# rsasaki0109/lidarslam_ros2

Hardware: AMD Instinct MI355X
Metric: scan registrations/sec (30k-pt scan vs 10-frame submap) (higher is better)
Workload: dtype f32; 1 GPU; cfg2: single NDT align(), 30000-pt VLP-32 scan (vg 0.2) vs 10-frame submap (vg 0.1), ndt_resolution 5.0, DIRECT7, max_iterations 30, transformation_epsilon 0; 1018 different scans (stream of 64); target_points=661519, voxels_valid=643, derivative_passes_last_scan=242, parallelism=1 registration stream per GPU x1, collective=none (one rank)

## Files before the change

include/lidarslam_reg.h:

```cpp
#ifndef LIDARSLAM_REG_H
#define LIDARSLAM_REG_H

#include <stddef.h>
#include <stdint.h>

#ifdef __cplusplus
extern "C" {
#endif

typedef struct lsr_handle_s* lsr_handle;

typedef enum lsr_status {
  LSR_OK = 0,
  LSR_ERR_INVALID_ARGUMENT = -1,
  LSR_ERR_NO_DEVICE = -2,
  LSR_ERR_HIP = -3,
  LSR_ERR_NO_TARGET = -4,
  LSR_ERR_NO_SOURCE = -5,
  LSR_ERR_NOT_IMPLEMENTED = -6,
  LSR_ERR_INDEX_OVERFLOW = -7,
  LSR_ERR_TOO_FEW_POINTS = -8
} lsr_status;

typedef enum lsr_method { LSR_METHOD_NDT = 0, LSR_METHOD_GICP = 1 } lsr_method;
// ... 129 lines not shown
  double distance;
  const void* cloud;
  size_t n_points;
} lsr_submap;
typedef struct lsr_loop_params {
  double threshold_loop_closure_score;
  double distance_loop_closure;
  double range_of_searching_loop_closure;
  int search_submap_num;
  float voxel_leaf_size;
  int top_k;
  int reserved;
} lsr_loop_params;
typedef struct lsr_loop_edge {
  int id_from;
  int id_to;
  int accepted;
  int converged;
  int iterations;
  int n_target_points;
  double candidate_distance;
  double fitness_score;
  double relative_pose[16];
  float final_transformation[16];
} lsr_loop_edge;
int lsr_search_loop(lsr_handle h, const lsr_submap* submaps, int num_submaps, size_t stride_bytes, int on_device,
                    const lsr_loop_params* params, lsr_loop_edge* edges, int edge_capacity, int* n_evaluated);

int lsr_ndt_grid_info(lsr_handle h, int32_t* info8);
int lsr_ndt_grid_dump(lsr_handle h, int32_t* idx, int32_t* npts, double* mean, double* icov);
int lsr_ndt_grid_centroids(lsr_handle h, float* centroid);
int lsr_ndt_derivatives(lsr_handle h, const double* p6, const float* T16, int compute_hessian, double* score,
                        double* grad, double* hess);
int lsr_gicp_covariances(lsr_handle h, int which, double* cov);
int lsr_nearest_neighbors(lsr_handle h, const float* T16, int32_t* idx, float* d2);
int lsr_get_profile(lsr_handle h, lsr_profile* out, int reset);
int lsr_debug_angle_tables(const double* p6, int d1_sign, float* jang_ref, float* hang_ref, float* jang_tab, float* hang_tab);

#ifdef __cplusplus
}
#endif
#endif
```

lidarslam_ros2_amd/_capi.py:

```python
from __future__ import annotations

import ctypes as C
import os

_HERE = os.path.dirname(os.path.abspath(__file__))
LIB_PATH = os.path.join(_HERE, os.environ.get("LSR_LIB_NAME", "liblidarslam_reg.so"))

OK = 0
METHOD_NDT, METHOD_GICP = 0, 1
KDTREE, DIRECT26, DIRECT7, DIRECT1 = 0, 1, 2, 3
(RESOLUTION, TRANSFORMATION_EPSILON, STEP_SIZE, OUTLIER_RATIO, MAX_CORRESPONDENCE_DISTANCE, ROTATION_EPSILON,
 EUCLIDEAN_FITNESS_EPSILON, GICP_EPSILON) = range(8)
(MAX_ITERATIONS, NEIGHBORHOOD, NUM_THREADS, K_CORRESPONDENCES, MAX_INNER_ITERATIONS, RANSAC_ITERATIONS,
 HESSIAN_D1_SIGN, PROFILE, NDT_WORKGROUP, NDT_TABLE_MODE, GRID_BUILDER, WAIT_MODE, NDT_QUAD, _UNASSIGNED_45, VOXEL_FILTER_FORM, NDT_SPLIT, TARGET_PREPARED) = range(32, 49)

EXPORTED_SYMBOLS = [
    "lsr_version", "lsr_status_string", "lsr_last_error", "lsr_device_count", "lsr_create", "lsr_destroy",
    "lsr_set_f64", "lsr_set_i32", "lsr_get_f64", "lsr_get_i32", "lsr_set_input_target", "lsr_set_input_target_device",
    "lsr_set_input_target_frames", "lsr_set_input_source", "lsr_set_input_source_device", "lsr_set_input_source_filtered", "lsr_set_input_source_frontend", "lsr_voxel_grid_filter",
    "lsr_share_target", "lsr_wait_stream", "lsr_align", "lsr_align_batch",
    "lsr_get_final_transformation", "lsr_has_converged", "lsr_get_fitness_score", "lsr_search_loop", "lsr_ndt_grid_info",
    "lsr_ndt_grid_dump", "lsr_ndt_grid_centroids", "lsr_ndt_derivatives", "lsr_gicp_covariances", "lsr_nearest_neighbors", "lsr_get_profile",
    "lsr_debug_angle_tables", "lsr_set_input_source_pc2", "lsr_get_source_pc2", "lsr_voxel_grid_filter_pc2", "lsr_shard_range", "lsr_comm_unique_id", "lsr_comm_create", "lsr_comm_destroy", "lsr_align_batch_sharded",
    "lsr_shard_plan", "lsr_align_batch_planned", "lsr_align_fitness_batch",
    "lsr_set_input_target_batch", "lsr_set_input_source_batch", "lsr_get_fitness_score_batch", "lsr_set_input_target_bcast", "lsr_get_source_pc2_device",
    "lsr_comm_all_gather_records", "lsr_set_input_target_frames_filtered", "lsr_prepare_target",
]


class Result(C.Structure):
    _fields_ = [("converged", C.c_int32), ("iterations", C.c_int32), ("score", C.c_double),
                ("n_evaluations", C.c_int32), ("n_correspondences", C.c_int32), ("gpu_ms", C.c_double)]


class Profile(C.Structure):
    _fields_ = [("deriv_ms_total", C.c_double), ("deriv_launches", C.c_int64), ("deriv_points", C.c_int64),
                ("deriv_pairs", C.c_int64)]


class SubMap(C.Structure):
    _fields_ = [("position", C.c_double * 3), ("orientation", C.c_double * 4), ("distance", C.c_double),
                ("cloud", C.c_void_p), ("n_points", C.c_size_t)]


class LoopParams(C.Structure):
    _fields_ = [("threshold_loop_closure_score", C.c_double), ("distance_loop_closure", C.c_double),
                ("range_of_searching_loop_closure", C.c_double), ("search_submap_num", C.c_int),
                ("voxel_leaf_size", C.c_float), ("top_k", C.c_int), ("reserved", C.c_int)]


class LoopEdge(C.Structure):
    _fields_ = [("id_from", C.c_int), ("id_to", C.c_int), ("accepted", C.c_int), ("converged", C.c_int),
                ("iterations", C.c_int), ("n_target_points", C.c_int), ("candidate_distance", C.c_double),
                ("fitness_score", C.c_double), ("relative_pose", C.c_double * 16), ("final_transformation", C.c_float * 16)]

# ... 39 lines not shown
    L.lsr_destroy.argtypes = [vp]
    L.lsr_set_f64.argtypes = [vp, C.c_int, C.c_double]
    L.lsr_set_i32.argtypes = [vp, C.c_int, C.c_int]
    L.lsr_get_f64.argtypes = [vp, C.c_int, dp]
    L.lsr_get_i32.argtypes = [vp, C.c_int, ip]
    for name in ("lsr_set_input_target", "lsr_set_input_target_device", "lsr_set_input_source",
                 "lsr_set_input_source_device"):
        getattr(L, name).argtypes = [vp, vp, C.c_size_t, C.c_size_t]
    L.lsr_share_target.argtypes = [vp, vp]
    L.lsr_wait_stream.argtypes = [vp, vp]
    L.lsr_set_input_target_frames.argtypes = [vp, C.c_int, C.POINTER(vp), C.POINTER(C.c_size_t), C.c_size_t, fp, C.c_int]
    L.lsr_set_input_target_frames_filtered.argtypes = [vp, C.c_int, C.POINTER(vp), C.POINTER(C.c_size_t), C.c_size_t, fp, C.c_int, C.c_float,
                                                       C.POINTER(C.c_size_t)]
    L.lsr_prepare_target.argtypes = [vp]
    L.lsr_set_input_source_filtered.argtypes = [vp, vp, C.c_size_t, C.c_size_t, C.c_float, C.c_int, C.POINTER(C.c_size_t)]
    L.lsr_set_input_source_frontend.argtypes = [vp, vp, C.c_size_t, C.c_size_t, C.c_double, C.c_double, C.c_float, C.c_int,
                                                C.POINTER(C.c_size_t)]
    L.lsr_voxel_grid_filter.argtypes = [vp, vp, C.c_size_t, C.c_size_t, C.c_float, vp, C.c_size_t, C.c_size_t,
                                        C.POINTER(C.c_size_t)]
    L.lsr_align.argtypes = [vp, fp, fp, C.POINTER(Result), vp, C.c_size_t]
    L.lsr_align_batch.argtypes = [C.POINTER(vp), C.c_int, fp, fp, C.POINTER(Result)]
    L.lsr_get_final_transformation.argtypes = [vp, fp]
    L.lsr_has_converged.argtypes = [vp, ip]
    L.lsr_get_fitness_score.argtypes = [vp, C.c_double, dp]
    L.lsr_get_fitness_score_batch.argtypes = [C.POINTER(vp), C.c_int, C.c_double, dp]
    L.lsr_set_input_target_batch.argtypes = [C.POINTER(vp), C.c_int, C.POINTER(vp), C.POINTER(C.c_size_t), C.c_size_t, C.c_int]
    L.lsr_set_input_source_batch.argtypes = [C.POINTER(vp), C.c_int, C.POINTER(vp), C.POINTER(C.c_size_t), C.c_size_t, C.c_int]
    L.lsr_search_loop.argtypes = [vp, C.POINTER(SubMap), C.c_int, C.c_size_t, C.c_int, C.POINTER(LoopParams),
                                  C.POINTER(LoopEdge), C.c_int, ip]
    L.lsr_ndt_grid_info.argtypes = [vp, ip]
    L.lsr_ndt_grid_dump.argtypes = [vp, ip, ip, dp, dp]
    L.lsr_ndt_grid_centroids.argtypes = [vp, fp]
    L.lsr_ndt_derivatives.argtypes = [vp, dp, fp, C.c_int, dp, dp, dp]
    L.lsr_gicp_covariances.argtypes = [vp, C.c_int, dp]
    L.lsr_nearest_neighbors.argtypes = [vp, fp, ip, fp]
    L.lsr_get_profile.argtypes = [vp, C.POINTER(Profile), C.c_int]
    L.lsr_debug_angle_tables.argtypes = [dp, C.c_int, fp, fp, fp, fp]
    L.lsr_set_input_source_pc2.argtypes = [vp, vp, C.c_size_t, C.POINTER(Pc2Layout), C.c_double, C.c_double, C.c_float, C.c_int,
                                           C.POINTER(C.c_size_t)]
    L.lsr_get_source_pc2.argtypes = [vp, vp, C.c_size_t, C.POINTER(Pc2Layout), C.POINTER(C.c_size_t)]
    L.lsr_get_source_pc2_device.argtypes = [vp, vp, C.c_size_t, C.POINTER(Pc2Layout), C.POINTER(C.c_size_t)]
    L.lsr_voxel_grid_filter_pc2.argtypes = [vp, vp, C.c_size_t, C.POINTER(Pc2Layout), C.c_float, vp, C.c_size_t, C.POINTER(Pc2Layout),
                                            C.POINTER(C.c_size_t)]
    L.lsr_shard_range.argtypes = [C.c_int, C.c_int, C.c_int, ip, ip]
    L.lsr_shard_range.restype = None
    L.lsr_comm_unique_id.argtypes = [vp]
    L.lsr_comm_create.argtypes = [vp, C.c_int, C.c_int, C.c_int, C.POINTER(vp)]
    L.lsr_comm_destroy.argtypes = [vp]
    L.lsr_align_batch_sharded.argtypes = [vp, C.POINTER(vp), C.c_int, C.c_int, fp, C.c_int, C.POINTER(ShardRecord)]
    L.lsr_set_input_target_bcast.argtypes = [vp, vp, vp, C.c_size_t, C.c_size_t, C.c_int, C.c_int]
    L.lsr_align_fitness_batch.argtypes = [C.POINTER(vp), C.c_int, fp, fp, C.POINTER(Result), C.c_double, dp]
    i32p = C.POINTER(C.c_int32)
    L.lsr_shard_plan.argtypes = [C.c_int, dp, C.c_int, i32p, i32p, i32p]
    L.lsr_align_batch_planned.argtypes = [vp, C.POINTER(vp), C.c_int, C.c_int, i32p, i32p, fp, C.c_int, C.POINTER(ShardRecord)]
    for name in EXPORTED_SYMBOLS:
        fn = getattr(L, name)
        if fn.restype is C.c_int or name not in ("lsr_version", "lsr_status_string", "lsr_last_error"):
            if name not in ("lsr_version", "lsr_status_string", "lsr_last_error", "lsr_shard_range"):
                fn.restype = C.c_int
    _lib = L
    return L


def check(status: int, where: str) -> None:
    if status != OK:
        raise RegistrationError(status, where)
# ... 1 lines not shown
```

lidarslam_ros2_amd/csrc/capi.hip:

```cpp
#include <algorithm>
#include <chrono>
#include <functional>
#include <limits>
#include <cmath>
#include <cstdlib>
#include <mutex>
#include <numeric>
#include <thread>

#include "handle.hpp"

namespace lsr {
static thread_local std::string g_last_error;
void set_last_error(const std::string& s) { g_last_error = s; }
}

using namespace lsr;

namespace {

#define LSR_CHECK_HANDLE(h)                      \
  if (!(h)) {                                    \
    set_last_error("null handle");               \
    return LSR_ERR_INVALID_ARGUMENT;             \
// ... 562 lines not shown
    return LSR_OK;
  };
  const std::function<int()> poll_hook = [&]() { return eager_dispatch(false); };
  int launches = 0;
  st = run_ndt_feeder(lead, lead->d_prob.p, lead->h_prob.p, cfg, min_evals, hard_cap, token, &launches, eager ? &poll_hook : nullptr,
                      !cfg.quad ? nb_full : 0, n_chains, chain_first, chain_streams);
  if (!chain_join.join() && !st) { set_last_error("joining a launch chain failed"); st = LSR_ERR_HIP; }
  if (eager && !st) st = eager_dispatch(true);
  if (eager) {
    (void)hipEventRecord(lead->side_ev, lead->side_stream);
    for (int b = 0; b < B; b++) {
      if (!eager_sent[b]) continue;
      double v = 0;
      const int fst = nn_fitness_end(hs[b]->scratch, lead->side_stream, &v);
      if (fst && !st) st = fst;
      if (!fst) fitness_out[b] = v;
    }
  }
  if (prefetched || eager) {
    if (hipEventSynchronize(lead->side_ev) != hipSuccess && !st) { set_last_error("side-stream work of the candidate set failed"); st = LSR_ERR_HIP; }
    if (st && prefetched) for (int b = 0; b < B; b++) if (hs[b]->target) hs[b]->target->has_hash = false;
  }
  if (st) return st;
  const double ms = std::chrono::duration<double, std::milli>(std::chrono::steady_clock::now() - t0).count();
  const NdtMailbox* M = lead->mailbox.p;
  if (lead->profile) {
    LSR_HIP(hipEventRecord(lead->ev1, lead->stream));
    LSR_HIP(hipEventSynchronize(lead->ev1));
    float ev_ms = 0.f;
    LSR_HIP(hipEventElapsedTime(&ev_ms, lead->ev0, lead->ev1));
    int passes = 0;
    lead->prof.deriv_pairs = 0;
    for (int b = 0; b < B; b++) {
      passes = std::max(passes, M[b].n_evals);
      lead->prof.deriv_pairs += (int64_t)M[b].last_pairs;
    }
    lead->prof.deriv_ms_total += ev_ms;
    lead->prof.deriv_launches += passes;
    lead->prof.deriv_points += (int64_t)passes * pts;
  }
  for (int b = 0; b < B; b++) {
    lsr_handle h = hs[b];
    std::memcpy(h->final_T, M[b].final_T, sizeof(float) * 16);
    h->converged = M[b].converged;
    if (finals) std::memcpy(finals + 16 * b, M[b].final_T, sizeof(float) * 16);
    if (results) {
      results[b].converged = M[b].converged;
      results[b].iterations = M[b].nr_iterations;
      results[b].score = M[b].trans_probability;
      results[b].n_evaluations = M[b].n_evals;
      results[b].n_correspondences = (int)M[b].last_pairs;
      results[b].gpu_ms = ms;
    }
  }
  return LSR_OK;
}

}

extern "C" {

const char* lsr_version(void) { return "lidarslam_reg 0.1.0 (gfx950)"; }

const char* lsr_status_string(int status) {
  switch (status) {
    case LSR_OK: return "ok";
    case LSR_ERR_INVALID_ARGUMENT: return "invalid argument";
// ... 1043 lines not shown
  if (!centroid) return LSR_ERR_INVALID_ARGUMENT;
  if (!h->target) return LSR_ERR_NO_TARGET;
  int st = ensure_ndt_grid(h);
  if (st) return st;
  TargetData& t = *h->target;
  {
    std::lock_guard<std::mutex> lock(t.build_mutex);
    if (!t.has_centroids && t.grid.ncells > 0) {
      if ((st = ndt_build_centroids(t.cloud, t.grid, h->scratch, h->stream))) return st;
      t.has_centroids = true;
    }
  }
  const VoxelGridDev& g = t.grid;
  const int L = g.n_leaves;
  if (L == 0) return LSR_OK;
  const size_t n_slots = g.dense ? g.ncells : (size_t)L;
  std::vector<int> keys(L), slot(g.ncells);
  std::vector<float> cen(n_slots * 4);
  LSR_HIP(hipMemcpy(keys.data(), g.leaf_key.p, sizeof(int) * L, hipMemcpyDeviceToHost));
  LSR_HIP(hipMemcpy(slot.data(), g.cell_slot.p, sizeof(int) * g.ncells, hipMemcpyDeviceToHost));
  LSR_HIP(hipMemcpy(cen.data(), g.centroid.p, sizeof(float) * 4 * n_slots, hipMemcpyDeviceToHost));
  int c = 0;
  for (int r = 0; r < L; r++) {
    if (keys[r] < 0) continue;
    const int s = kd_slot(slot[(size_t)keys[r]]);
    for (int k = 0; k < 3; k++) centroid[c * 3 + k] = (s >= 0) ? cen[(size_t)s * 4 + k] : std::numeric_limits<float>::quiet_NaN();
    c++;
  }
  return LSR_OK;
}

int lsr_ndt_derivatives(lsr_handle h, const double* p6, const float* T16, int compute_hessian, double* score, double* grad,
                        double* hess) {
  LSR_CHECK_HANDLE(h);
  if (!p6) return LSR_ERR_INVALID_ARGUMENT;
  if (!h->target || h->target->n == 0) return LSR_ERR_NO_TARGET;
  if (!h->has_source) return LSR_ERR_NO_SOURCE;
  int st = ensure_ndt_grid(h);
  if (st) return st;
  if (h->target->grid.ncells == 0) { set_last_error("the input target holds no finite point"); return LSR_ERR_NO_TARGET; }
  if ((st = h->d_state.reserve(2))) return st;
  if ((st = h->h_state.reserve(2, hipHostMallocMapped))) return st;
  if ((st = h->d_prob.reserve(1))) return st;
  if ((st = h->h_prob.reserve(1, hipHostMallocMapped))) return st;
  NdtLaunchCfg cfg;
  cfg.neighborhood = h->ndt.neighborhood;
  {
    lsr_handle one[1] = {h};
    choose_table_mode(h, one, 1, cfg);
  }
  if ((st = h->d_bins.reserve((size_t)NDT_NBANKS * NDT_BANK_WORDS))) return st;
  LSR_HIP(hipMemsetAsync(h->d_bins.p, 0, sizeof(long long) * NDT_NBANKS * NDT_BANK_WORDS, h->stream));
  cfg.max_blocks = ndt_nblocks(h->source.n, h->device, 1, cfg_wg_threads(cfg), cfg_wg_points(cfg));
  ndt_fill_diag_state(h->h_state.p[0], p6, T16, compute_hessian, h->ndt, (int)h->source.n);
  h->h_state.p[1] = h->h_state.p[0];
  fill_problem(h->h_prob.p[0], h, h->d_state.p, h->d_bins.p, cfg);
  LSR_HIP(hipMemcpyAsync(h->d_prob.p, h->h_prob.p, sizeof(NdtProblem), hipMemcpyHostToDevice, h->stream));
  LSR_HIP(hipMemcpyAsync(h->d_state.p, h->h_state.p, 2 * sizeof(NdtState), hipMemcpyHostToDevice, h->stream));
  if ((st = ndt_launch_evals(h->d_prob.p, h->h_prob.p, cfg, 0, 2, h->stream))) return st;
  LSR_HIP(hipMemcpyAsync(h->h_state.p, h->d_state.p, sizeof(NdtState), hipMemcpyDeviceToHost, h->stream));
  LSR_HIP(hipStreamSynchronize(h->stream));
  const NdtState& S = h->h_state.p[0];
  if (score) *score = S.score;
  if (grad) for (int i = 0; i < 6; i++) grad[i] = S.g[i];
  if (hess) for (int i = 0; i < 36; i++) hess[i] = compute_hessian ? S.H[i] : 0.0;
  return LSR_OK;
}

int lsr_gicp_covariances(lsr_handle h, int which, double* cov) {
  LSR_CHECK_HANDLE(h);
  if (!cov) return LSR_ERR_INVALID_ARGUMENT;
  return gicp_get_covariances(h, which, cov);
}

int lsr_get_profile(lsr_handle h, lsr_profile* out, int reset) {
  LSR_CHECK_HANDLE(h);
  if (out) *out = h->prof;
  if (reset) h->prof = lsr_profile{0, 0, 0, 0};
  return LSR_OK;
}

}
```

lidarslam_ros2_amd/csrc/ndt.hip:

```cpp
#include "ndt.hpp"

#include <cmath>
#include <cstdlib>
#include <type_traits>

#include "grid_device.hpp"
#include "ndt_point.hpp"
#include "sort.hpp"

namespace lsr {

namespace {

__host__ __device__ inline void angle_tables(const double* p, bool with_hessian, int d1_sign, float* jang, float* hang) {
  double cx, cy, cz, sx, sy, sz;
  if (fabs(p[3]) < 10e-5) { cx = 1.0; sx = 0.0; } else { cx = cos(p[3]); sx = sin(p[3]); }
  if (fabs(p[4]) < 10e-5) { cy = 1.0; sy = 0.0; } else { cy = cos(p[4]); sy = sin(p[4]); }
  if (fabs(p[5]) < 10e-5) { cz = 1.0; sz = 0.0; } else { cz = cos(p[5]); sz = sin(p[5]); }
  jang[0] = (float)(-sx * sz + cx * sy * cz); jang[1] = (float)(-sx * cz - cx * sy * sz); jang[2] = (float)(-cx * cy);
  jang[3] = (float)(cx * sz + sx * sy * cz);  jang[4] = (float)(cx * cz - sx * sy * sz);  jang[5] = (float)(-sx * cy);
  jang[6] = (float)(-sy * cz);                jang[7] = (float)(sy * sz);                 jang[8] = (float)(cy);
  jang[9] = (float)(sx * cy * cz);            jang[10] = (float)(-sx * cy * sz);          jang[11] = (float)(sx * sy);
  jang[12] = (float)(-cx * cy * cz);          jang[13] = (float)(cx * cy * sz);           jang[14] = (float)(-cx * sy);
  jang[15] = (float)(-cy * sz);               jang[16] = (float)(-cy * cz);               jang[17] = 0.f;
// ... 58 lines not shown
void ndt_fill_initial_state(NdtState& st, const float* guess16 , const NdtParamsHost& prm, int n_points) {
  std::memset(&st, 0, sizeof(st));
  ndt_fill_align_constants(st, prm, n_points);
  float I16[16] = {1, 0, 0, 0, 0, 1, 0, 0, 0, 0, 1, 0, 0, 0, 0, 1};
  const float* G = guess16 ? guess16 : I16;
  std::memcpy(st.final_T, G, sizeof(I16));
  st.T[0] = G[0]; st.T[1] = G[4]; st.T[2] = G[8];  st.T[3] = G[12];
  st.T[4] = G[1]; st.T[5] = G[5]; st.T[6] = G[9];  st.T[7] = G[13];
  st.T[8] = G[2]; st.T[9] = G[6]; st.T[10] = G[10]; st.T[11] = G[14];
  float e[3];
  euler012_f(G, e);
  st.p[0] = G[12]; st.p[1] = G[13]; st.p[2] = G[14];
  st.p[3] = e[0]; st.p[4] = e[1]; st.p[5] = e[2];
  for (int i = 0; i < 6; i++) st.x_t[i] = st.p[i];
  angle_tables(st.p, true, st.d1_sign, st.jang, st.hang);
  st.want_hessian = 1;
  st.phase = PH_INIT;
  st.done = 0;
}

void ndt_fill_diag_state(NdtState& st, const double* p6, const float* T16, int compute_hessian, const NdtParamsHost& prm,
                         int n_points) {
  std::memset(&st, 0, sizeof(st));
  ndt_fill_align_constants(st, prm, n_points);
  for (int i = 0; i < 6; i++) st.p[i] = st.x_t[i] = p6[i];
  if (T16) {
    st.T[0] = T16[0]; st.T[1] = T16[4]; st.T[2] = T16[8];  st.T[3] = T16[12];
    st.T[4] = T16[1]; st.T[5] = T16[5]; st.T[6] = T16[9];  st.T[7] = T16[13];
    st.T[8] = T16[2]; st.T[9] = T16[6]; st.T[10] = T16[10]; st.T[11] = T16[14];
  } else {
    pose_to_T12(p6, st.T);
  }
  angle_tables(p6, true, st.d1_sign, st.jang, st.hang);
  st.want_hessian = compute_hessian ? 1 : 0;
  st.phase = PH_DIAG;
}

namespace {

__device__ __forceinline__ double wave_sum(double v) {
#pragma unroll
  for (int m = 32; m >= 1; m >>= 1) v += __shfl_xor(v, m, 64);
  return v;
}

typedef __attribute__((address_space(3))) NdtState LdsState;
typedef __attribute__((address_space(3))) double LdsDouble;

__device__ __forceinline__ double mt_div(double a, double b) {
  if (!(fabs(b) > 1e-290 && fabs(b) < 1e290)) return a / b;
  double r = __builtin_amdgcn_rcp(b);
  r = fma(fma(-b, r, 1.0), r, r);
  r = fma(fma(-b, r, 1.0), r, r);
  const double q = a * r;
  return fma(fma(-b, q, a), r, q);
}
__device__ __forceinline__ double mt_sqrt(double x) {
  if (!(x > 1e-290 && x < 1e290)) return sqrt(x);
  double y = __builtin_amdgcn_rsq(x);
  y = y * fma(-0.5 * x * y, y, 1.5);
  y = y * fma(-0.5 * x * y, y, 1.5);
  const double s = x * y;
  return fma(fma(-s, s, x), 0.5 * y, s);
}

__device__ __forceinline__ double mt_trial_value(double a_l, double f_l, double g_l, double a_u, double f_u, double g_u, double a_t,
                                 double f_t, double g_t) {
// ... 209 lines not shown
    cs_f[lane] = sn;
  } else if (lane == 6) {
    f[0] = 1.0;
    f[7] = 0.0;
  }
  wave_lds_fence();
  const bool with_hang = (mode & 2) != 0;
  if (lane < 24 || with_hang) {
    double val = angle_entry_value(ent_a, f);
    if (lane == 24 + 20 && S->d1_sign < 0) val = -val;
    if (lane < 24) S->jang[lane] = (float)val; else S->hang[lane - 24] = (float)val;
  }
  if (with_hang && lane < 8) S->hang[40 + lane] = (float)angle_entry_value(ent_b, f);
  if (lane == 63) {
    float* T = S->T;
    compose_R12(cs_f[0], cs_f[1], cs_f[2], cs_f[3], cs_f[4], cs_f[5], T);
    T[3] = (float)S->x_t[0]; T[7] = (float)S->x_t[1]; T[11] = (float)S->x_t[2];
    T12_to_colmajor16(T, S->final_T);
  }
  if (lane == 0) S->pad1 = 0;
  wave_lds_fence();
}

enum CtlNext : int { CTL_DONE = 0, CTL_NEWTON_BEGIN = 1, CTL_NEWTON_END = 2 };

__device__ __forceinline__ int ndt_controller_mt(LdsState* S, const LdsDouble* sums) {
  const double mu = 1.e-4, nu = 0.9;
  const int max_step_iterations = 10;
  double sv[8];
#pragma unroll
  for (int k = 0; k < 8; k++) sv[k] = sums[k];
  const int phase = S->phase;
  const bool had_hessian = S->want_hessian != 0;
  const int n_evals = S->n_evals + 1;
  if (phase == PH_INIT || phase == PH_MT_HESS || phase == PH_DIAG) {
    S->n_evals = n_evals;
    S->last_pairs = sv[7];
    if (phase != PH_MT_HESS) {
      S->score = sv[0];
#pragma unroll
      for (int i = 0; i < 6; i++) S->g[i] = sv[1 + i];
    }
    if (phase == PH_DIAG) {
      if (had_hessian) {
        double hu[21];
#pragma unroll
        for (int k = 0; k < 21; k++) hu[k] = sums[8 + k];
        int k = 0;
#pragma unroll
        for (int i = 0; i < 6; i++)
#pragma unroll
          for (int j = i; j < 6; j++) {
            S->H[i * 6 + j] = hu[k];
            S->H[j * 6 + i] = hu[k];
            k++;
          }
      }
      S->done = 1;
      return CTL_DONE;
    }
    return phase == PH_INIT ? CTL_NEWTON_BEGIN : CTL_NEWTON_END;
  }
  int open_interval = S->open_interval, interval_converged = S->interval_converged, step_iterations = S->step_iterations;
  const double step_max = S->step_max, step_min = S->step_min;
  double p[6], dir[6];
#pragma unroll
  for (int i = 0; i < 6; i++) { p[i] = S->p[i]; dir[i] = S->dir[i]; }
  const double phi_0 = S->phi_0, d_phi_0 = S->d_phi_0;
  double a_t = S->a_t;
  MtInterval I = {S->a_l, S->f_l, S->g_l, S->a_u, S->f_u, S->g_u};

  const double score = sv[0];
  const double phi_t = -score;
  double dot = 0;
#pragma unroll
  for (int i = 0; i < 6; i++) dot += sv[1 + i] * dir[i];
  const double d_phi_t = -dot;
  const double psi_t = phi_t - phi_0 - mu * d_phi_0 * a_t;
  const double d_psi_t = d_phi_t - mu * d_phi_0;
  if (phase == PH_MT_TRIAL) {
    if (open_interval && (psi_t <= 0 && d_psi_t >= 0)) {
      open_interval = 0;
      I.f_l = I.f_l + phi_0 - mu * d_phi_0 * I.a_l;
      I.g_l = I.g_l + mu * d_phi_0;
      I.f_u = I.f_u + phi_0 - mu * d_phi_0 * I.a_u;
      I.g_u = I.g_u + mu * d_phi_0;
    }
    if (open_interval)
      interval_converged = mt_update_interval(I, a_t, psi_t, d_psi_t) ? 1 : 0;
    else
      interval_converged = mt_update_interval(I, a_t, phi_t, d_phi_t) ? 1 : 0;
    step_iterations++;
  }
  int next = CTL_DONE;
  if (!interval_converged && step_iterations < max_step_iterations && !(psi_t <= 0 && d_phi_t <= -nu * d_phi_0)) {
    if (open_interval)
      a_t = mt_trial_value(I.a_l, I.f_l, I.g_l, I.a_u, I.f_u, I.g_u, a_t, psi_t, d_psi_t);
    else
      a_t = mt_trial_value(I.a_l, I.f_l, I.g_l, I.a_u, I.f_u, I.g_u, a_t, phi_t, d_phi_t);
    a_t = fmax(fmin(a_t, step_max), step_min);
#pragma unroll
    for (int i = 0; i < 6; i++) S->x_t[i] = p[i] + dir[i] * a_t;
    S->a_t = a_t;
    S->want_hessian = 0;
    S->phase = PH_MT_TRIAL;
    S->pad1 = 1;
  } else if (step_iterations) {
    S->want_hessian = 1;
    S->phase = PH_MT_HESS;
  } else {
    next = CTL_NEWTON_END;
  }
  S->n_evals = n_evals;
  S->last_pairs = sv[7];
  S->score = score;
#pragma unroll
  for (int i = 0; i < 6; i++) S->g[i] = sv[1 + i];
  S->open_interval = open_interval;
  S->interval_converged = interval_converged;
  S->step_iterations = step_iterations;
  S->a_l = I.a_l; S->f_l = I.f_l; S->g_l = I.g_l; S->a_u = I.a_u; S->f_u = I.f_u; S->g_u = I.g_u;
  return next;
}

__device__ __forceinline__ int ndt_newton_end(LdsState* S) {
  const int nr_iterations = S->nr_iterations, max_iter = S->max_iter;
  const double a_t = S->a_t, eps = S->eps;
  double p[6], dir[6];
#pragma unroll
  for (int i = 0; i < 6; i++) { p[i] = S->p[i]; dir[i] = S->dir[i]; }
  const double score = S->score;
  const int n_points = S->n_points;
  int converged = S->converged;
  if (nr_iterations > max_iter || (nr_iterations && (fabs(a_t) < eps))) converged = 1;
#pragma unroll
  for (int i = 0; i < 6; i++) S->p[i] = p[i] + dir[i] * a_t;
  S->nr_iterations = nr_iterations + 1;
  S->converged = converged;
  if (converged) {
    S->trans_probability = score / (double)n_points;
    S->done = 1;
    return CTL_DONE;
  }
  return CTL_NEWTON_BEGIN;
}

// ... 308 lines not shown
  if (tid < 64) {
    if (seq > 0) {
      if (tid < NDT_NRED) {
        double t = (((s_bin[4][tid] + s_bin[3][tid]) + s_bin[2][tid]) + s_bin[1][tid]) + s_bin[0][tid];
        if (s_bin[0][31] != 0.0 || s_bin[1][31] != 0.0) t = __longlong_as_double(0x7FF8000000000000ll);
        s_sum[tid] = t;
      }
      wave_lds_fence();
      LSR_STAMP(6)
      LSR_CTL_BEGIN(L)
      ndt_controller_wave0(L, (const LdsDouble*)s_sum);
      wave_lds_fence();
      LSR_CTL_END(0)
      LSR_STAMP(5)
      build_request_wave0(reinterpret_cast<NdtState*>(s_state), &s_lu[0][0], reinterpret_cast<float*>(&s_lu[4][0]), ang_entry, ang_entry_b);
      LSR_CTL_END(2)
      LSR_STAMP(4)
    }
    if (blockIdx.x == 0) {
      uint4* gq = reinterpret_cast<uint4*>(Sout);
      gq[tid] = s_state_q[tid];
      if (tid + 64 < STATE_Q) gq[tid + 64] = s_state_q[tid + 64];
    }
  }
  __syncthreads();
  if (uniform_i(L->done)) {
    if (P.mailbox != nullptr && blockIdx.x == 0 && tid == 0) {
      NdtMailbox* mb = P.mailbox;
#pragma unroll
      for (int k = 0; k < 16; k++) mb->final_T[k] = L->final_T[k];
      mb->converged = L->converged;
      mb->nr_iterations = L->nr_iterations;
      mb->n_evals = L->n_evals;
      mb->trans_probability = L->trans_probability;
      mb->last_pairs = L->last_pairs;
      __threadfence_system();
      __hip_atomic_store(&mb->done, (unsigned int)L->token, __ATOMIC_RELEASE, __HIP_MEMORY_SCOPE_SYSTEM);
    }
    return;
  }
  if (blockIdx.x == 0) {
    uint4* zb = reinterpret_cast<uint4*>(P.bins + (size_t)((seq + 1) % NDT_NBANKS) * NDT_BANK_WORDS);
    for (int k = tid; k < NDT_BANK_WORDS / 2; k += THREADS) zb[k] = make_uint4(0u, 0u, 0u, 0u);
  }
  LSR_STAMP(7)
  LSR_PASS_MARK(_p_t7)

  const bool hess = uniform_i(L->want_hessian) != 0;
  const double d1d = uniform_d(L->d1);
  const float d2 = uniform_f((float)L->d2);
  float T[12];
#pragma unroll
  for (int k = 0; k < 12; k++) T[k] = uniform_f(L->T[k]);
  const float leaf = P.leaf;
  LSR_STAMP(11)

  const unsigned short* s_map = reinterpret_cast<const unsigned short*>(s_table);
  const float4* s_rec = reinterpret_cast<const float4*>(reinterpret_cast<const unsigned char*>(s_table) + P.lds_map_bytes);

  long long* const bank = P.bins + (size_t)(seq % NDT_NBANKS) * NDT_BANK_WORDS + (size_t)(blockIdx.x & (NDT_NSHARDS - 1)) * (NDT_NBINS * 32);
  const bool one_batch = (long long)blockIdx.x * PTS + stride >= (long long)P.n;
  for (int base = blockIdx.x * PTS; base < P.n; base += stride) {
    {
      const float tx = xform_ref(T[0], T[1], T[2], T[3], x, y, z);
      const float ty = xform_ref(T[4], T[5], T[6], T[7], x, y, z);
      const float tz = xform_ref(T[8], T[9], T[10], T[11], x, y, z);
      const float fx = floorf(tx / leaf), fy = floorf(ty / leaf), fz = floorf(tz / leaf);
      const bool finite_ok = (i < P.n) && (fabsf(fx) < 1.0e9f) && (fabsf(fy) < 1.0e9f) && (fabsf(fz) < 1.0e9f);
      const int ci = finite_ok ? (int)fx : INT_MIN / 2, cj = finite_ok ? (int)fy : INT_MIN / 2, ck = finite_ok ? (int)fz : INT_MIN / 2;

      bool valid[NT], score_only[NT];
      int cellv[NT];
#pragma unroll
      for (int t = 0; t < NT; t++) {
        score_only[t] = false;
        const int o = ql + 4 * t;
        int dx, dy, dz;
        Offsets<NOFF>::get(o, dx, dy, dz);
        const int a = ci + dx, b = cj + dy, c = ck + dz;
        const bool in = (o < NOFF) & (a >= P.min_b[0]) & (a <= P.max_b[0]) & (b >= P.min_b[1]) & (b <= P.max_b[1]) &
                        (c >= P.min_b[2]) & (c <= P.max_b[2]);
// ... 76 lines not shown
        if (npairs != 0.f) {
          point_terms(false, x, y, z, score, npairs, A0, A1, A2, 0.f, 0.f, 0.f, 0.f, 0.f, 0.f, L->jang, L->hang, o);
        } else {
#pragma unroll
          for (int k = 0; k < NDT_NRED_GRAD; k++) o[k] = 0.f;
        }
        s_o[ql][pq] = (ql == 0) ? o[0] : (ql == 1) ? o[1] : (ql == 2) ? o[2] : o[3];
        s_o[4 + ql][pq] = (ql == 0) ? o[4] : (ql == 1) ? o[5] : (ql == 2) ? o[6] : o[7];
      }
      i += stride;
      x = 0.f; y = 0.f; z = 0.f;
      if (i < P.n) { x = P.sx[i]; y = P.sy[i]; z = P.sz[i]; }
    }
    LSR_STAMP(12)
    barrier_lds_only();
    if (hess) {
      if (tid < PTS) {
        const float npairs = s_pt[1][tid];
        float o[29];
        if (npairs != 0.f) {
          point_terms(true, s_pt[11][tid], s_pt[12][tid], s_pt[13][tid], s_pt[0][tid], npairs, s_pt[2][tid], s_pt[3][tid], s_pt[4][tid],
                      s_pt[5][tid], s_pt[6][tid], s_pt[7][tid], s_pt[8][tid], s_pt[9][tid], s_pt[10][tid], L->jang, L->hang, o);
        } else {
#pragma unroll
          for (int k = 0; k < 29; k++) o[k] = 0.f;
        }
#pragma unroll
        for (int k = 0; k < 29; k++) s_o[k][tid] = o[k];
      }
      LSR_STAMP(13)
      barrier_lds_only();
    }
    LSR_STAMP(14)
    if (!hess) {
      constexpr int RUNS = PTS / 8;
      if (tid < NDT_NRED_GRAD * RUNS) {
        const int v = tid / RUNS, k = tid & 7;
        const double t = canon::reduce_grad(&s_o[v][8 * (tid % RUNS)]);
        bool poison;
        long long m = canon::piece(t, k < NDT_NBINS ? k : 0, &poison);
        int pz = poison ? 1 : 0;
        if (PTS == 128) { m += (long long)__shfl_xor((int)m, 8, 64); pz |= __shfl_xor(pz, 8, 64); }
        if ((tid & (RUNS - 1)) < NDT_NBINS) {
          unsigned long long* dst = one_batch ? reinterpret_cast<unsigned long long*>(bank) : s_ibin;
          if (m != 0) atomicAdd(dst + k * 32 + v, (unsigned long long)m);
          if (pz && k == 0) atomicAdd(dst + 31, 1ull);
        }
      }
    } else {
      constexpr int RUNS = PTS / 16;
      if (tid < ((29 * RUNS + 63) & ~63)) {
        const int v = tid / RUNS, sg = tid & 3;
        double t = 0.0;
        if (v < 29) t = canon::reduce_hess(&s_o[v][16 * (tid % RUNS)]);
        bool poison, poison0;
        long long m = canon::piece(t, sg + 1, &poison);
        long long m0 = canon::piece(t, 0, &poison0);
        int pz = poison0 ? 1 : 0;
        if (PTS == 128) {
          m += (long long)__shfl_xor((int)m, 4, 64); m0 += (long long)__shfl_xor((int)m0, 4, 64); pz |= __shfl_xor(pz, 4, 64);
        }
        if (v < 29 && (tid & (RUNS - 1)) < 4) {
          unsigned long long* dst = one_batch ? reinterpret_cast<unsigned long long*>(bank) : s_ibin;
          if (m != 0) atomicAdd(dst + (sg + 1) * 32 + v, (unsigned long long)m);
          if (sg == 0) {
            if (m0 != 0) atomicAdd(dst + v, (unsigned long long)m0);
            if (pz) atomicAdd(dst + 31, 1ull);
          }
        }
      }
    }
    if (!hess && base + stride < P.n) barrier_lds_only();
  }

  LSR_STAMP(2)
  LSR_PASS_MARK(_p_t2)
  if (!one_batch) {
    __syncthreads();
    if (tid < NDT_NBINS * 32) {
      const unsigned long long m = s_ibin[tid];
      if (m != 0ull) atomicAdd(reinterpret_cast<unsigned long long*>(bank + tid), m);
    }
  }
  LSR_STAMP(3)
  LSR_PASS_END(hess)
// ... 75 lines not shown
    unsigned char* dst = reinterpret_cast<unsigned char*>(s_table);
    if (tid >= 64)
      for (int c = wave - 1; c < nchunks; c += NWAVES - 1)
        __builtin_amdgcn_global_load_lds((const __attribute__((address_space(1))) void*)(img + (size_t)c * 1024),
                                         (__attribute__((address_space(3))) void*)(dst + (size_t)c * 1024), 16, 0, 0);
  }
  if (tid < 64) {
    if (seq > 0) {
      if (tid < NDT_NRED) {
        double t = (((s_bin[4][tid] + s_bin[3][tid]) + s_bin[2][tid]) + s_bin[1][tid]) + s_bin[0][tid];
        if (s_bin[0][31] != 0.0 || s_bin[1][31] != 0.0) t = __longlong_as_double(0x7FF8000000000000ll);
        s_sum[tid] = t;
      }
      wave_lds_fence();
      ndt_controller_wave0(L, (const LdsDouble*)s_sum);
      wave_lds_fence();
      build_request_wave0(reinterpret_cast<NdtState*>(s_state), &s_lu[0][0], reinterpret_cast<float*>(&s_lu[4][0]), ang_entry, ang_entry_b);
    }
    if (blockIdx.x == 0) {
      uint4* gq = reinterpret_cast<uint4*>(Sout);
      gq[tid] = s_state_q[tid];
      if (tid + 64 < STATE_Q) gq[tid + 64] = s_state_q[tid + 64];
    }
  }
  __syncthreads();
  if (uniform_i(L->done)) {
    if (P.mailbox != nullptr && blockIdx.x == 0 && tid == 0) {
      NdtMailbox* mb = P.mailbox;
#pragma unroll
      for (int k = 0; k < 16; k++) mb->final_T[k] = L->final_T[k];
      mb->converged = L->converged;
      mb->nr_iterations = L->nr_iterations;
      mb->n_evals = L->n_evals;
      mb->trans_probability = L->trans_probability;
      mb->last_pairs = L->last_pairs;
      __threadfence_system();
      __hip_atomic_store(&mb->done, (unsigned int)L->token, __ATOMIC_RELEASE, __HIP_MEMORY_SCOPE_SYSTEM);
    }
    return;
  }
  if (blockIdx.x == 0) {
    uint4* zb = reinterpret_cast<uint4*>(P.bins + (size_t)((seq + 1) % NDT_NBANKS) * NDT_BANK_WORDS);
    for (int k = tid; k < NDT_BANK_WORDS / 2; k += THREADS) zb[k] = make_uint4(0u, 0u, 0u, 0u);
  }

  const bool hess = uniform_i(L->want_hessian) != 0;
  const double d1d = uniform_d(L->d1);
  const float d2 = uniform_f((float)L->d2);
  float T[12];
#pragma unroll
  for (int k = 0; k < 12; k++) T[k] = uniform_f(L->T[k]);
  const float leaf = P.leaf;
  const int mb0 = P.min_b[0], mb1 = P.min_b[1], mb2 = P.min_b[2];
  const int xb0 = P.max_b[0], xb1 = P.max_b[1], xb2 = P.max_b[2];
  const int mul1 = P.mul1, mul2 = P.mul2;
  const __attribute__((address_space(3))) unsigned short* s_map = (const __attribute__((address_space(3))) unsigned short*)s_table;
  const int map_bytes = P.lds_map_bytes;
  float* s_tile = reinterpret_cast<float*>(reinterpret_cast<unsigned char*>(s_table) + tab_bytes) + wave * canon::TILE_FLOATS;
  const GlbV4* g_rec = (const GlbV4*)P.rec;
  const GlbInt* g_cell_slot = (const GlbInt*)P.cell_slot;
  const GlbFloat* g_sx = (const GlbFloat*)P.sx;
  const GlbFloat* g_sy = (const GlbFloat*)P.sy;
  const GlbFloat* g_sz = (const GlbFloat*)P.sz;
  (void)g_rec; (void)g_cell_slot; (void)s_map; (void)map_bytes;

  for (int base = SPLIT ? blockIdx.x * PTS : blockIdx.x * PTS + cw * 64; base < n; base += stride) {
    const bool have = i < n;
    const float px = x, py = y, pz = z;
    const float tx = xform_ref(T[0], T[1], T[2], T[3], px, py, pz);
    const float ty = xform_ref(T[4], T[5], T[6], T[7], px, py, pz);
    const float tz = xform_ref(T[8], T[9], T[10], T[11], px, py, pz);
    i += stride;
    if (i < n) { x = g_sx[i]; y = g_sy[i]; z = g_sz[i]; }
    const float fx = floorf(tx / leaf), fy = floorf(ty / leaf), fz = floorf(tz / leaf);
    const bool finite_ok = have && (fabsf(fx) < 1.0e9f) && (fabsf(fy) < 1.0e9f) && (fabsf(fz) < 1.0e9f);
    const int ci = finite_ok ? (int)fx : INT_MIN / 2, cj = finite_ok ? (int)fy : INT_MIN / 2, ck = finite_ok ? (int)fz : INT_MIN / 2;
    bool inx[3], iny[3], inz[3];
#pragma unroll
    for (int d = 0; d < 3; d++) {
// ... 103 lines not shown
#pragma unroll
        for (int k = 0; k < 11; k++) s_tile[k * canon::TILE_PITCH + lane] = S[k];
      }
      __syncthreads();
      if (role == 1) {
        if (base + stride < n) __syncthreads();
        continue;
      }
      const float* other = s_tile + canon::TILE_FLOATS;
#pragma unroll
      for (int k = 0; k < 11; k++) S[k] = S[k] + other[k * canon::TILE_PITCH + lane];
      if (base + stride < n) __syncthreads();
    }
    float o[29];
    {
      const bool any_pair = S[1] != 0.f;
      const float qx = any_pair ? px : 0.f, qy = any_pair ? py : 0.f, qz = any_pair ? pz : 0.f;
      point_terms(hess, qx, qy, qz, S[0], S[1], S[2], S[3], S[4], S[5], S[6], S[7], S[8], S[9], S[10], L->jang, L->hang, o);
    }
    if (!hess) {
#pragma unroll
      for (int k = 0; k < NDT_NRED_GRAD; k++) s_tile[k * canon::TILE_PITCH + lane] = o[k];
      wave_lds_fence();
      const int v = lane >> 3, g = lane & 7;
      const double t = canon::reduce_grad(s_tile + v * canon::TILE_PITCH + 8 * g);
      if (g < NDT_NBINS) canon::add_piece_lds(s_ibin, v, g, t);
    } else {
#pragma unroll
      for (int r = 0; r < 2; r++) {
#pragma unroll
        for (int k = 0; k < 16; k++)
          if (16 * r + k < 29) s_tile[k * canon::TILE_PITCH + lane] = o[16 * r + k];
        wave_lds_fence();
        const int v = 16 * r + (lane >> 2), sg = lane & 3;
        const double t = canon::reduce_hess(s_tile + (lane >> 2) * canon::TILE_PITCH + 16 * sg);
        if (v < 29) {
          canon::add_piece_lds(s_ibin, v, sg + 1, t);
          if (sg == 0) canon::add_piece_lds(s_ibin, v, 0, t);
        }
      }
    }
  }

  __syncthreads();
  if (tid < NDT_NBINS * 32) {
    const unsigned long long m = s_ibin[tid];
    if (m != 0ull) {
      long long* bank = P.bins + (size_t)(seq % NDT_NBANKS) * NDT_BANK_WORDS + (size_t)(blockIdx.x & (NDT_NSHARDS - 1)) * (NDT_NBINS * 32);
      atomicAdd(reinterpret_cast<unsigned long long*>(bank + tid), m);
    }
  }
}

#ifdef LSR_TIMING
}
extern "C" int lsr_debug_timing_buffer(long long** out) {
  static long long* buf = nullptr;
  if (!buf) {
    if (hipMalloc((void**)&buf, 1024 * 32 * sizeof(long long)) != hipSuccess) return -1;
    (void)hipMemset(buf, 0, 1024 * 32 * sizeof(long long));
    (void)hipMemcpyToSymbol(HIP_SYMBOL(g_lsr_timing), &buf, sizeof(buf));
  }
  *out = buf;
  return 0;
}
namespace {
#endif

}
// ... 175 lines not shown
```

lidarslam_ros2_amd/csrc/ndt.hpp:

```cpp
#pragma once
#include "common.hpp"

namespace lsr {

enum NdtPhase : int {
  PH_INIT = 0,
  PH_MT_FIRST = 1,
  PH_MT_TRIAL = 2,
  PH_MT_HESS = 3,
  PH_DIAG = 4
};

constexpr int NDT_NRED = 32;
constexpr int NDT_NRED_GRAD = 8;
constexpr int NDT_LANE_THREADS = 512;
constexpr int NDT_MAX_BLOCKS = 1024;
constexpr int ndt_lane_tile_bytes(int threads) { return (threads / 64) * 16 * 68 * 4; }
constexpr int NDT_LDS_REC_BYTES = 48;
constexpr int NDT_LDS_TABLE_MAX = 128 * 1024;
constexpr int NDT_LDS_TABLE_MAX_QUAD = 120 * 1024;

constexpr int NDT_NBINS = 5;
constexpr int NDT_NSHARDS = 8;
constexpr int NDT_BANK_WORDS = NDT_NSHARDS * NDT_NBINS * 32;
constexpr int NDT_NBANKS = 3;

enum NdtTableMode : int {
  NDT_TAB_DENSE = 0,
  NDT_TAB_COMPACT = 1,
  NDT_TAB_LDS = 2
};

__host__ __device__ inline int cell_slot_code(bool usable, int n, int slot) { return usable ? slot : (n < 0 ? -2 - slot : -1); }
__host__ __device__ inline int kd_slot(int code) { return code >= -1 ? code : -2 - code; }

struct NdtState {
  float T[12];
  float jang[24];
  float hang[48];
  int want_hessian;
  int done;
  int phase;
  int d1_sign;
  double d1, d2;
  double step_max, step_min, eps;
  int max_iter, n_points;
  double p[6], x_t[6], dir[6];
  double score, g[6], H[36];
  int nr_iterations, converged;
  double phi_0, d_phi_0, a_l, f_l, g_l, a_u, f_u, g_u, a_t;
  int open_interval, interval_converged, step_iterations;
  int token;
  float final_T[16];
  double trans_probability;
  double last_pairs;
  int n_evals, pad1;
};

struct NdtMailbox {
  unsigned long long progress;
  unsigned int done;
  int converged, nr_iterations, n_evals;
  double trans_probability, last_pairs;
  float final_T[16];
};

struct NdtProblem {
  const float* sx;
  const float* sy;
  const float* sz;
  int n;
  int nblocks;
  const int* cell_slot;
  const float4* rec;
  int min_b[3];
  int max_b[3];
  int mul1, mul2;
  float leaf;
  int lds_map_bytes;
  const uint4* lds_image;
  int lds_bytes;
  long long* bins;
  NdtState* st;
  NdtMailbox* mailbox;
  const float4* centroid;
  float radius2;
};

struct NdtParamsHost {
  double resolution = 1.0, step_size = 0.1, outlier_ratio = 0.55, trans_eps = 0.1;
  int max_iterations = 35;
  int neighborhood = LSR_DIRECT7;
  int d1_sign = 1;
};

void ndt_gauss_constants(double resolution, double outlier_ratio, double* d1, double* d2);

// ... 64 lines not shown
```

lidarslam_ros2_amd/registration.py:

```python
from __future__ import annotations

import ctypes as C
from typing import Optional, Sequence

import numpy as np

from . import _capi as capi

DIRECT7, DIRECT1, DIRECT26, KDTREE = capi.DIRECT7, capi.DIRECT1, capi.DIRECT26, capi.KDTREE


def _is_torch_cuda(x) -> bool:
    return hasattr(x, "is_cuda") and bool(x.is_cuda)


def _cloud_args(cloud, reg=None):
    if _is_torch_cuda(cloud):
        import torch

        t = cloud
        if t.dtype != torch.float32 or t.dim() != 2 or t.shape[1] < 3:
            raise ValueError("device cloud must be float32 of shape (n, c>=3)")
        if not t.is_contiguous():
            t = t.contiguous()
# ... 316 lines not shown

    def setNeighborhoodSearchMethod(self, method: int):
        self._seti(capi.NEIGHBORHOOD, method, "setNeighborhoodSearchMethod")

    def setNumThreads(self, n: int):
        self._seti(capi.NUM_THREADS, n, "setNumThreads")

    def setHessianD1Sign(self, sign: int):
        self._seti(capi.HESSIAN_D1_SIGN, sign, "setHessianD1Sign")

    def getTransformationProbability(self) -> float:
        return float(self._last.score)

    def gridInfo(self) -> dict:
        info = np.zeros(8, np.int32)
        capi.check(self._lib.lsr_ndt_grid_info(self._h, info.ctypes.data_as(C.POINTER(C.c_int32))), "gridInfo")
        return dict(min_b=info[0:3].copy(), max_b=info[3:6].copy(), n_leaves=int(info[6]), n_valid=int(info[7]))

    def gridDump(self) -> dict:
        n = self.gridInfo()["n_leaves"]
        idx, npts = np.zeros(n, np.int32), np.zeros(n, np.int32)
        mean, icov = np.zeros((n, 3)), np.zeros((n, 3, 3))
        capi.check(self._lib.lsr_ndt_grid_dump(self._h, idx.ctypes.data_as(C.POINTER(C.c_int32)),
                                               npts.ctypes.data_as(C.POINTER(C.c_int32)),
                                               mean.ctypes.data_as(C.POINTER(C.c_double)),
                                               icov.ctypes.data_as(C.POINTER(C.c_double))), "gridDump")
        return dict(idx=idx, n=npts, mean=mean, icov=icov)

    def gridCentroids(self) -> np.ndarray:
        c = np.zeros((self.gridInfo()["n_leaves"], 3), np.float32)
        capi.check(self._lib.lsr_ndt_grid_centroids(self._h, c.ctypes.data_as(C.POINTER(C.c_float))), "gridCentroids")
        return c

    def derivatives(self, p, T=None, compute_hessian: bool = True):
        p = np.ascontiguousarray(p, np.float64)
        t = _mat_to_col16(T) if T is not None else None
        score = C.c_double()
        g, H = np.zeros(6), np.zeros((6, 6))
        capi.check(self._lib.lsr_ndt_derivatives(self._h, p.ctypes.data_as(C.POINTER(C.c_double)),
                                                 t.ctypes.data_as(C.POINTER(C.c_float)) if t is not None else None,
                                                 1 if compute_hessian else 0, C.byref(score),
                                                 g.ctypes.data_as(C.POINTER(C.c_double)),
                                                 H.ctypes.data_as(C.POINTER(C.c_double))), "derivatives")
        return score.value, g, H


class GeneralizedIterativeClosestPoint(Registration):

    _method = capi.METHOD_GICP

    def setRotationEpsilon(self, eps: float):
        self._setf(capi.ROTATION_EPSILON, eps, "setRotationEpsilon")

    def setCorrespondenceRandomness(self, k: int):
        self._seti(capi.K_CORRESPONDENCES, k, "setCorrespondenceRandomness")

    def setMaximumOptimizerIterations(self, n: int):
        self._seti(capi.MAX_INNER_ITERATIONS, n, "setMaximumOptimizerIterations")

    def covariances(self, which: str, raw: bool = False) -> np.ndarray:
        w = (0 if which == "source" else 1) + (2 if raw else 0)
        n = self._n_source if w in (0, 2) else self._n_target
        cov = np.zeros((n, 3, 3))
        capi.check(self._lib.lsr_gicp_covariances(self._h, w, cov.ctypes.data_as(C.POINTER(C.c_double))), "covariances")
        return cov

    def setInputTarget(self, cloud):
        super().setInputTarget(cloud)
        self._n_target = int(np.shape(cloud)[0]) if not _is_torch_cuda(cloud) else int(cloud.shape[0])


def set_input_target_batch(regs: Sequence[Registration], clouds):
    lib = capi.load()
    B = len(regs)
    if len(clouds) != B:
        raise ValueError("one cloud per registration object")
# ... 80 lines not shown
```

Baseline: 440.2 registrations/s.

## Fuse last line-search trial gradient with Hessian pass in NDT More-Thuente

```diff
diff --git a/include/lidarslam_reg.h b/include/lidarslam_reg.h
--- a/include/lidarslam_reg.h
+++ b/include/lidarslam_reg.h
@@ -185,6 +185,8 @@
 int lsr_ndt_grid_centroids(lsr_handle h, float* centroid);
 int lsr_ndt_derivatives(lsr_handle h, const double* p6, const float* T16, int compute_hessian, double* score,
                         double* grad, double* hess);
+int lsr_ndt_derivatives_pairs(lsr_handle h, const double* p6, const float* T16, int compute_hessian, double* score,
+                              double* grad, double* hess, double* pairs);
 int lsr_gicp_covariances(lsr_handle h, int which, double* cov);
 int lsr_nearest_neighbors(lsr_handle h, const float* T16, int32_t* idx, float* d2);
 int lsr_get_profile(lsr_handle h, lsr_profile* out, int reset);
diff --git a/lidarslam_ros2_amd/_capi.py b/lidarslam_ros2_amd/_capi.py
--- a/lidarslam_ros2_amd/_capi.py
+++ b/lidarslam_ros2_amd/_capi.py
@@ -20,7 +20,7 @@
     "lsr_set_input_target_frames", "lsr_set_input_source", "lsr_set_input_source_device", "lsr_set_input_source_filtered", "lsr_set_input_source_frontend", "lsr_voxel_grid_filter",
     "lsr_share_target", "lsr_wait_stream", "lsr_align", "lsr_align_batch",
     "lsr_get_final_transformation", "lsr_has_converged", "lsr_get_fitness_score", "lsr_search_loop", "lsr_ndt_grid_info",
-    "lsr_ndt_grid_dump", "lsr_ndt_grid_centroids", "lsr_ndt_derivatives", "lsr_gicp_covariances", "lsr_nearest_neighbors", "lsr_get_profile",
+    "lsr_ndt_grid_dump", "lsr_ndt_grid_centroids", "lsr_ndt_derivatives", "lsr_ndt_derivatives_pairs", "lsr_gicp_covariances", "lsr_nearest_neighbors", "lsr_get_profile",
     "lsr_debug_angle_tables", "lsr_set_input_source_pc2", "lsr_get_source_pc2", "lsr_voxel_grid_filter_pc2", "lsr_shard_range", "lsr_comm_unique_id", "lsr_comm_create", "lsr_comm_destroy", "lsr_align_batch_sharded",
     "lsr_shard_plan", "lsr_align_batch_planned", "lsr_align_fitness_batch",
     "lsr_set_input_target_batch", "lsr_set_input_source_batch", "lsr_get_fitness_score_batch", "lsr_set_input_target_bcast", "lsr_get_source_pc2_device",
@@ -126,6 +126,7 @@
     L.lsr_ndt_grid_dump.argtypes = [vp, ip, ip, dp, dp]
     L.lsr_ndt_grid_centroids.argtypes = [vp, fp]
     L.lsr_ndt_derivatives.argtypes = [vp, dp, fp, C.c_int, dp, dp, dp]
+    L.lsr_ndt_derivatives_pairs.argtypes = [vp, dp, fp, C.c_int, dp, dp, dp, dp]
     L.lsr_gicp_covariances.argtypes = [vp, C.c_int, dp]
     L.lsr_nearest_neighbors.argtypes = [vp, fp, ip, fp]
     L.lsr_get_profile.argtypes = [vp, C.POINTER(Profile), C.c_int]
diff --git a/lidarslam_ros2_amd/csrc/capi.hip b/lidarslam_ros2_amd/csrc/capi.hip
--- a/lidarslam_ros2_amd/csrc/capi.hip
+++ b/lidarslam_ros2_amd/csrc/capi.hip
@@ -618,7 +618,7 @@
     int passes = 0;
     lead->prof.deriv_pairs = 0;
     for (int b = 0; b < B; b++) {
-      passes = std::max(passes, M[b].n_evals);
+      passes = std::max(passes, M[b].n_passes);
       lead->prof.deriv_pairs += (int64_t)M[b].last_pairs;
     }
     lead->prof.deriv_ms_total += ev_ms;
@@ -1728,8 +1728,13 @@
 
 int lsr_ndt_derivatives(lsr_handle h, const double* p6, const float* T16, int compute_hessian, double* score, double* grad,
                         double* hess) {
-  LSR_CHECK_HANDLE(h);
-  if (!p6) return LSR_ERR_INVALID_ARGUMENT;
+  return lsr_ndt_derivatives_pairs(h, p6, T16, compute_hessian, score, grad, hess, nullptr);
+}
+
+int lsr_ndt_derivatives_pairs(lsr_handle h, const double* p6, const float* T16, int compute_hessian, double* score, double* grad,
+                              double* hess, double* pairs) {
+  LSR_CHECK_HANDLE(h);
+  if (!p6 || compute_hessian < 0 || compute_hessian > 2) return LSR_ERR_INVALID_ARGUMENT;
   if (!h->target || h->target->n == 0) return LSR_ERR_NO_TARGET;
   if (!h->has_source) return LSR_ERR_NO_SOURCE;
   int st = ensure_ndt_grid(h);
@@ -1760,6 +1765,7 @@
   if (score) *score = S.score;
   if (grad) for (int i = 0; i < 6; i++) grad[i] = S.g[i];
   if (hess) for (int i = 0; i < 36; i++) hess[i] = compute_hessian ? S.H[i] : 0.0;
+  if (pairs) *pairs = S.last_pairs;
   return LSR_OK;
 }
 
diff --git a/lidarslam_ros2_amd/csrc/ndt.hip b/lidarslam_ros2_amd/csrc/ndt.hip
--- a/lidarslam_ros2_amd/csrc/ndt.hip
+++ b/lidarslam_ros2_amd/csrc/ndt.hip
@@ -114,7 +114,7 @@
     pose_to_T12(p6, st.T);
   }
   angle_tables(p6, true, st.d1_sign, st.jang, st.hang);
-  st.want_hessian = compute_hessian ? 1 : 0;
+  st.want_hessian = compute_hessian == 2 ? NDT_PASS_FUSED : (compute_hessian ? NDT_PASS_HESS : NDT_PASS_GRAD);
   st.phase = PH_DIAG;
 }
 
@@ -390,9 +390,11 @@
   for (int k = 0; k < 8; k++) sv[k] = sums[k];
   const int phase = S->phase;
   const bool had_hessian = S->want_hessian != 0;
-  const int n_evals = S->n_evals + 1;
+  const int n_evals = S->n_evals + (phase == PH_MT_LAST ? 2 : 1);
+  const int n_passes = S->n_passes + 1;
   if (phase == PH_INIT || phase == PH_MT_HESS || phase == PH_DIAG) {
     S->n_evals = n_evals;
+    S->n_passes = n_passes;
     S->last_pairs = sv[7];
     if (phase != PH_MT_HESS) {
       S->score = sv[0];
@@ -436,7 +438,7 @@
   const double d_phi_t = -dot;
   const double psi_t = phi_t - phi_0 - mu * d_phi_0 * a_t;
   const double d_psi_t = d_phi_t - mu * d_phi_0;
-  if (phase == PH_MT_TRIAL) {
+  if (phase == PH_MT_TRIAL || phase == PH_MT_LAST) {
     if (open_interval && (psi_t <= 0 && d_psi_t >= 0)) {
       open_interval = 0;
       I.f_l = I.f_l + phi_0 - mu * d_phi_0 * I.a_l;
@@ -460,9 +462,12 @@
 #pragma unroll
     for (int i = 0; i < 6; i++) S->x_t[i] = p[i] + dir[i] * a_t;
     S->a_t = a_t;
-    S->want_hessian = 0;
-    S->phase = PH_MT_TRIAL;
+    const bool last = step_iterations + 1 >= max_step_iterations;
+    S->want_hessian = last ? NDT_PASS_FUSED : NDT_PASS_GRAD;
+    S->phase = last ? PH_MT_LAST : PH_MT_TRIAL;
     S->pad1 = 1;
+  } else if (phase == PH_MT_LAST) {
+    next = CTL_NEWTON_END;
   } else if (step_iterations) {
     S->want_hessian = 1;
     S->phase = PH_MT_HESS;
@@ -470,6 +475,7 @@
     next = CTL_NEWTON_END;
   }
   S->n_evals = n_evals;
+  S->n_passes = n_passes;
   S->last_pairs = sv[7];
   S->score = score;
 #pragma unroll
@@ -844,6 +850,7 @@
       mb->converged = L->converged;
       mb->nr_iterations = L->nr_iterations;
       mb->n_evals = L->n_evals;
+      mb->n_passes = L->n_passes;
       mb->trans_probability = L->trans_probability;
       mb->last_pairs = L->last_pairs;
       __threadfence_system();
@@ -858,7 +865,9 @@
   LSR_STAMP(7)
   LSR_PASS_MARK(_p_t7)
 
-  const bool hess = uniform_i(L->want_hessian) != 0;
+  const int form = uniform_i(L->want_hessian);
+  const bool hess = form != NDT_PASS_GRAD;
+  const bool fused = form == NDT_PASS_FUSED;
   const double d1d = uniform_d(L->d1);
   const float d2 = uniform_f((float)L->d2);
   float T[12];
@@ -1001,7 +1010,7 @@
       barrier_lds_only();
     }
     LSR_STAMP(14)
-    if (!hess) {
+    if (!hess || fused) {
       constexpr int RUNS = PTS / 8;
       if (tid < NDT_NRED_GRAD * RUNS) {
         const int v = tid / RUNS, k = tid & 7;
@@ -1016,10 +1025,15 @@
           if (pz && k == 0) atomicAdd(dst + 31, 1ull);
         }
       }
-    } else {
+    }
+    if (hess) {
       constexpr int RUNS = PTS / 16;
-      if (tid < ((29 * RUNS + 63) & ~63)) {
-        const int v = tid / RUNS, sg = tid & 3;
+      static_assert(NDT_NRED_GRAD * (PTS / 8) % 64 == 0 && NDT_NRED_GRAD * (PTS / 8) + (((29 - NDT_NRED_GRAD) * RUNS + 63) & ~63) <= THREADS,
+                    "fused pass: the two trees sit on whole waves of their own");
+      const int v0 = fused ? NDT_NRED_GRAD : 0;
+      const int ht = tid - (fused ? NDT_NRED_GRAD * (PTS / 8) : 0);
+      if (ht >= 0 && ht < (((29 - v0) * RUNS + 63) & ~63)) {
+        const int v = v0 + ht / RUNS, sg = tid & 3;
         double t = 0.0;
         if (v < 29) t = canon::reduce_hess(&s_o[v][16 * (tid % RUNS)]);
         bool poison, poison0;
@@ -1161,6 +1175,7 @@
       mb->converged = L->converged;
       mb->nr_iterations = L->nr_iterations;
       mb->n_evals = L->n_evals;
+      mb->n_passes = L->n_passes;
       mb->trans_probability = L->trans_probability;
       mb->last_pairs = L->last_pairs;
       __threadfence_system();
@@ -1173,7 +1188,9 @@
     for (int k = tid; k < NDT_BANK_WORDS / 2; k += THREADS) zb[k] = make_uint4(0u, 0u, 0u, 0u);
   }
 
-  const bool hess = uniform_i(L->want_hessian) != 0;
+  const int form = uniform_i(L->want_hessian);
+  const bool hess = form != NDT_PASS_GRAD;
+  const bool fused = form == NDT_PASS_FUSED;
   const double d1d = uniform_d(L->d1);
   const float d2 = uniform_f((float)L->d2);
   float T[12];
@@ -1343,9 +1360,14 @@
         for (int k = 0; k < 16; k++)
           if (16 * r + k < 29) s_tile[k * canon::TILE_PITCH + lane] = o[16 * r + k];
         wave_lds_fence();
+        if (fused && r == 0) {
+          const int vg = lane >> 3, g = lane & 7;
+          const double tg = canon::reduce_grad(s_tile + vg * canon::TILE_PITCH + 8 * g);
+          if (g < NDT_NBINS) canon::add_piece_lds(s_ibin, vg, g, tg);
+        }
         const int v = 16 * r + (lane >> 2), sg = lane & 3;
         const double t = canon::reduce_hess(s_tile + (lane >> 2) * canon::TILE_PITCH + 16 * sg);
-        if (v < 29) {
+        if (v < 29 && !(fused && v < NDT_NRED_GRAD)) {
           canon::add_piece_lds(s_ibin, v, sg + 1, t);
           if (sg == 0) canon::add_piece_lds(s_ibin, v, 0, t);
         }
diff --git a/lidarslam_ros2_amd/csrc/ndt.hpp b/lidarslam_ros2_amd/csrc/ndt.hpp
--- a/lidarslam_ros2_amd/csrc/ndt.hpp
+++ b/lidarslam_ros2_amd/csrc/ndt.hpp
@@ -8,7 +8,14 @@
   PH_MT_FIRST = 1,
   PH_MT_TRIAL = 2,
   PH_MT_HESS = 3,
-  PH_DIAG = 4
+  PH_DIAG = 4,
+  PH_MT_LAST = 5
+};
+
+enum NdtPassForm : int {
+  NDT_PASS_GRAD = 0,
+  NDT_PASS_HESS = 1,
+  NDT_PASS_FUSED = 2
 };
 
 constexpr int NDT_NRED = 32;
@@ -55,7 +62,10 @@
   double trans_probability;
   double last_pairs;
   int n_evals, pad1;
+  int n_passes;
+  int pad2[3];
 };
+static_assert(sizeof(NdtState) % 16 == 0 && sizeof(NdtState) <= 128 * 16, "NdtState travels as at most 128 uint4");
 
 struct NdtMailbox {
   unsigned long long progress;
@@ -63,6 +73,7 @@
   int converged, nr_iterations, n_evals;
   double trans_probability, last_pairs;
   float final_T[16];
+  int n_passes;
 };
 
 struct NdtProblem {
diff --git a/lidarslam_ros2_amd/registration.py b/lidarslam_ros2_amd/registration.py
--- a/lidarslam_ros2_amd/registration.py
+++ b/lidarslam_ros2_amd/registration.py
@@ -372,16 +372,19 @@
         capi.check(self._lib.lsr_ndt_grid_centroids(self._h, c.ctypes.data_as(C.POINTER(C.c_float))), "gridCentroids")
         return c
 
-    def derivatives(self, p, T=None, compute_hessian: bool = True):
+    def derivatives(self, p, T=None, compute_hessian=True, with_pairs: bool = False):
         p = np.ascontiguousarray(p, np.float64)
         t = _mat_to_col16(T) if T is not None else None
-        score = C.c_double()
+        score, pairs = C.c_double(), C.c_double()
         g, H = np.zeros(6), np.zeros((6, 6))
-        capi.check(self._lib.lsr_ndt_derivatives(self._h, p.ctypes.data_as(C.POINTER(C.c_double)),
-                                                 t.ctypes.data_as(C.POINTER(C.c_float)) if t is not None else None,
-                                                 1 if compute_hessian else 0, C.byref(score),
-                                                 g.ctypes.data_as(C.POINTER(C.c_double)),
-                                                 H.ctypes.data_as(C.POINTER(C.c_double))), "derivatives")
+        form = 2 if (compute_hessian is not True and compute_hessian == 2) else (1 if compute_hessian else 0)
+        capi.check(self._lib.lsr_ndt_derivatives_pairs(self._h, p.ctypes.data_as(C.POINTER(C.c_double)),
+                                                       t.ctypes.data_as(C.POINTER(C.c_float)) if t is not None else None,
+                                                       form, C.byref(score),
+                                                       g.ctypes.data_as(C.POINTER(C.c_double)),
+                                                       H.ctypes.data_as(C.POINTER(C.c_double)), C.byref(pairs)), "derivatives")
+        if with_pairs:
+            return score.value, g, H, pairs.value
         return score.value, g, H
 
 
```

Result: faster. 463.7 registrations/s, median of 6 (+5.3%).
